# mcahny/vps

Measured on NVIDIA H100. Metric: FuseTrack frame pairs/s on synthetic 1024x2048 pairs, higher is better.
Workload: dtype f32 (wgmma: 3 split-f16 products per MAC, fp32 accumulate promoted to RN register sums)

## Files before the change

vps_b200/csrc/conv_tc32.cu:

```cuda
#include "conv_tc_common.cuh"

namespace {

constexpr int T32_CONV_WARPS = 3;
constexpr int T32_KC = 32;
constexpr int T32_MAX_N = 128;
constexpr int T32_WIDE_MAX_N = 64;
constexpr int t32_threads(int nwg) { return 128 * (nwg + 1); }
constexpr int T32_STAGE_SLOTS = 2;
constexpr int T32_PLANES = 2;

__device__ unsigned int g_tc32_overflow = 0;

struct Tc32Extra {
  int rows;
  int plane_bytes;
  int stage_bytes;
  int b_plane_bytes;
  int dcn;
  int dcn_split_n;
};

constexpr int DCN32_THREADS = 512;
constexpr int DCN32_GATHER_WARPS = 7;
constexpr int DCN32_MAX_N = 128;
constexpr int DCN32_LO_REGS = 80, DCN32_HI_REGS = 176;
static_assert(128 * (2 * DCN32_LO_REGS + 2 * DCN32_HI_REGS) == DCN32_THREADS * (65536 / DCN32_THREADS),
              "the DCN register split must use exactly the launch allocation");
static_assert(DCN32_LO_REGS % 8 == 0 && DCN32_HI_REGS % 8 == 0 && DCN32_LO_REGS >= 24 && DCN32_HI_REGS <= 256,
              "setmaxnreg counts are multiples of 8 in [24, 256]");

struct Ring32 {
  uint32_t s_base, s_bytes;
  uint32_t a_base, a_bytes;
  uint32_t b_base, b_bytes;
  uint32_t e_base, bias_base;
  uint32_t setup_base;
  uint32_t bar_base;
  uint32_t smem;
  __device__ __forceinline__ uint32_t sfull(int s) const { return bar_base + 8u * s; }
  __device__ __forceinline__ uint32_t sempty(int s) const { return bar_base + 8u * (MAX_STAGES + s); }
  __device__ __forceinline__ uint32_t pfull(int s) const { return bar_base + 8u * (2 * MAX_STAGES + s); }
  __device__ __forceinline__ uint32_t pempty(int s) const { return bar_base + 8u * (3 * MAX_STAGES + s); }
  __device__ __forceinline__ uint32_t bfull(int s) const { return bar_base + 8u * (4 * MAX_STAGES + s); }
  __device__ __forceinline__ uint32_t bempty(int s) const { return bar_base + 8u * (5 * MAX_STAGES + s); }
  __device__ __forceinline__ uint32_t unit_ctr() const { return bar_base + 8u * (6 * MAX_STAGES); }
  __device__ __forceinline__ uint32_t rfull(int wg) const { return bar_base + 8u * (6 * MAX_STAGES + 1 + wg); }
};
constexpr int T32_NBAR = 6 * MAX_STAGES;
constexpr int T32_BAR_BYTES = 8 * (T32_NBAR + 2 + 4);
constexpr int t32_box_c(int n) { return n >= 32 ? 32 : 16; }
constexpr int T32_EPI_MAX_N = 64;

__host__ __device__ __forceinline__ Ring32 ring32(uint32_t base, const ConvTcParams& p, const Tc32Extra& e, int nwg, bool epi_tma,
                                                  bool dcn) {
  Ring32 rg;
  rg.s_base = base; rg.s_bytes = dcn ? 0u : (uint32_t)e.stage_bytes;
  rg.a_base = rg.s_base + T32_STAGE_SLOTS * rg.s_bytes; rg.a_bytes = (uint32_t)T32_PLANES * (uint32_t)e.plane_bytes;
  rg.b_base = rg.a_base + (uint32_t)p.a_stages * rg.a_bytes; rg.b_bytes = (uint32_t)T32_PLANES * (uint32_t)e.b_plane_bytes;
  rg.e_base = rg.b_base + (uint32_t)p.b_stages * rg.b_bytes;
  rg.bias_base = rg.e_base + (epi_tma ? 64u * nwg * (uint32_t)p.block_n * 4u : 0u);
  rg.setup_base = rg.bias_base + (epi_tma ? (uint32_t)nwg * (uint32_t)p.block_n * 4u : 0u);
  rg.bar_base = rg.setup_base + (dcn ? (uint32_t)dcn_setup_bytes(e.rows) : 0u);
  rg.smem = rg.bar_base + T32_BAR_BYTES + 1024u - base;
  return rg;
}

struct Tc32Walk {
  int chunks, taps, kw;
  bool halo;
  __host__ __device__ __forceinline__ int steps() const { return chunks * taps; }
  __host__ __device__ __forceinline__ int items() const { return chunks * (halo ? 1 : taps); }
  __device__ __forceinline__ bool opens_item(int tap) const { return !halo || tap == 0; }
};
__host__ __device__ __forceinline__ Tc32Walk tc32_walk(const ConvTcParams& p) { return {p.cin_chunks, p.kh * p.kw, p.kw, p.halo != 0}; }

__device__ __forceinline__ void producer32(const ConvTcParams& p, const Tc32Extra& e, const Ring32& rg, const CUtensorMap* tmA,
                                           const CUtensorMap* tmB) {
  const Tc32Walk walk = tc32_walk(p);
  const uint32_t a_box_bytes = (uint32_t)p.a_box_bytes, b_bytes = (uint32_t)T32_PLANES * (uint32_t)e.b_plane_bytes;
  const int bn = p.block_n;
  RingPos sp, bp;
  for (int tile = blockIdx.x; tile < p.total_tiles; tile += gridDim.x) {
    const TileCoord t = tile_coord(p, tile);
    const int x_base = t.tx * p.tw * p.sw - p.pw_[t.prob];
    const int y_base = t.ty * p.th * p.sh - p.ph_[t.prob];
    const int n0 = t.n_idx * bn;
    for (int cc = 0; cc < walk.chunks; ++cc) {
      for (Tap tap; tap.k < walk.taps; tap.next(walk.kw)) {
        if (!e.dcn && walk.opens_item(tap.k)) {
          sp.wait_empty(rg.sempty(sp.slot));
          if (elect_one()) {
            mbar_expect_tx(rg.sfull(sp.slot), a_box_bytes);
            tma_load_4d(rg.s_base + sp.slot * rg.s_bytes, tmA, rg.sfull(sp.slot), cc * T32_KC,
                        walk.halo ? x_base : x_base + tap.s, walk.halo ? y_base : y_base + tap.r, t.img);
// ... 102 lines not shown
          acc[4] += wq[c] * v1[c].x; acc[5] += wq[c] * v1[c].y; acc[6] += wq[c] * v1[c].z; acc[7] += wq[c] * v1[c].w;
        }
        uint32_t hp[4], lp[4];
        bool over = false;
#pragma unroll
        for (int q = 0; q < 4; ++q) split_pair_f16(acc[2 * q], acc[2 * q + 1], hp[q], lp[q], over);
        if (over) atomicAdd(&g_tc32_overflow, 1u);
        const uint32_t off = (uint32_t)r * 64u + ((((uint32_t)j) ^ ((uint32_t)(r >> 1) & 3u)) << 4);
        const uint32_t pm = dst + off, pl = pm + (uint32_t)e.plane_bytes;
        asm volatile("st.shared.v4.b32 [%0], {%1, %2, %3, %4};" ::"r"(pm), "r"(hp[0]), "r"(hp[1]), "r"(hp[2]), "r"(hp[3]) : "memory");
        asm volatile("st.shared.v4.b32 [%0], {%1, %2, %3, %4};" ::"r"(pl), "r"(lp[0]), "r"(lp[1]), "r"(lp[2]), "r"(lp[3]) : "memory");
      }
      asm volatile("fence.proxy.async.shared::cta;" ::: "memory");
      __syncwarp();
      if (lane == 0) mbar_arrive(rg.pfull(ap.slot));
    }
    step_base += (uint32_t)steps_per_tile;
    asm volatile("bar.sync 1, %0;" ::"n"(NT) : "memory");
  }
}

template <int N>
__device__ __forceinline__ uint32_t epi_box_addr(uint32_t box, int q, int c) {
  constexpr int BC = t32_box_c(N);
  const uint32_t k = (uint32_t)((c % BC) >> 2);
  const uint32_t sw = BC == 32 ? (uint32_t)(q & 7) : (uint32_t)((q >> 1) & 3);
  return box + (uint32_t)(c / BC) * (64u * BC * 4u) + (uint32_t)q * (BC * 4u) + ((k ^ sw) << 4) + (uint32_t)(c & 3) * 4u;
}

struct EpiBox {
  int n0, x0, y0, img;
  bool live;
};
__device__ __forceinline__ EpiBox epi_box(const ConvTcParams& p, int tile, int wg) {
  const TileCoord t = tile_coord(p, tile);
  EpiBox b;
  b.n0 = t.n_idx * p.block_n; b.img = t.img;
  b.x0 = t.tx * p.tw + (64 * wg) % p.tw; b.y0 = t.ty * p.th + (64 * wg) / p.tw;
  b.live = b.x0 < p.ow && b.y0 < p.oh;
  return b;
}

template <int N>
__device__ __forceinline__ void epi_tma32(const ConvTcParams& p, const CUtensorMap* tmY, const float (&d)[N / 2], uint32_t box,
                                          uint32_t bias_s, float bias_v, uint32_t rbar, uint32_t rphase, int wg, int tile) {
  constexpr int BC = t32_box_c(N);
  const int i = threadIdx.x & 127, lane = threadIdx.x & 31, w = i >> 5;
  if (i < N) asm volatile("st.shared.f32 [%0], %1;" ::"r"(bias_s + 4u * i), "f"(bias_v) : "memory");
  if (i == 0) asm volatile("cp.async.bulk.wait_group.read 0;" ::: "memory");
  asm volatile("bar.sync %0, 128;" ::"r"(1 + wg) : "memory");
  if (p.res) mbar_wait(rbar, rphase);
#pragma unroll
  for (int h = 0; h < 2; ++h) {
    const int q = 16 * w + (lane >> 2) + 8 * h;
#pragma unroll
    for (int j = 0; j < N / 8; ++j) {
      const int c = 8 * j + 2 * (lane & 3);
      const uint32_t a = epi_box_addr<N>(box, q, c);
      float b0, b1, r0 = 0.f, r1 = 0.f;
      asm volatile("ld.shared.v2.f32 {%0, %1}, [%2];" : "=f"(b0), "=f"(b1) : "r"(bias_s + 4u * c));
      if (p.res) asm volatile("ld.shared.v2.f32 {%0, %1}, [%2];" : "=f"(r0), "=f"(r1) : "r"(a));
      const float2 v = epi_math(p, d[4 * j + 2 * h], d[4 * j + 2 * h + 1], b0, b1, r0, r1);
      asm volatile("st.shared.v2.f32 [%0], {%1, %2};" ::"r"(a), "f"(v.x), "f"(v.y) : "memory");
    }
  }
  asm volatile("fence.proxy.async.shared::cta;" ::: "memory");
  asm volatile("bar.sync %0, 128;" ::"r"(1 + wg) : "memory");
  const EpiBox eb = epi_box(p, tile, wg);
  if (i == 0 && eb.live) {
#pragma unroll
    for (int b = 0; b < N / BC; ++b) tma_store_4d(tmY, box + (uint32_t)b * (64u * BC * 4u), eb.n0 + b * BC, eb.x0, eb.y0, eb.img);
    asm volatile("cp.async.bulk.commit_group;" ::: "memory");
  }
}

template <int N, bool TMA_EPI>
__device__ __forceinline__ void consumer32(const ConvTcParams& p, const Tc32Extra& e, const Ring32& rg, int wg, int row0,
                                           uint32_t b_off, int c_off, const CUtensorMap* tmY, const CUtensorMap* tmR) {
  constexpr int BC = t32_box_c(N);
  const bool leader = (threadIdx.x & 127) == 0;
  constexpr bool epi_tma = TMA_EPI;
  const uint32_t box = rg.e_base + (uint32_t)wg * (64u * N * 4u), bias_s = rg.bias_base + (uint32_t)wg * (N * 4u);
  const uint32_t rbar = rg.rfull(wg);
  uint32_t rphase = 0;
  const bool halo = p.halo != 0;
  const int ntaps = p.kh * p.kw, kw = p.kw, last_cc = p.cin_chunks - 1;
  const uint32_t a_pitch = halo ? (uint32_t)p.halo_w * 64u : 512u;
  const uint64_t a_hi = desc_hi(64u, a_pitch), b_hi = desc_hi(64u, 512u);
  const uint32_t a_wg = halo ? (uint32_t)(row0 >> 3) * a_pitch : (uint32_t)row0 * 64u;
  const uint32_t plane = (uint32_t)e.plane_bytes, b_plane = (uint32_t)e.b_plane_bytes;
  float acc[N / 2], sum[N / 2];
  RingPos ap, bp;
  for (int tile = blockIdx.x; tile < p.total_tiles; tile += gridDim.x) {
    float bias_v = 0.f;
    if (epi_tma) {
      const int c = tile_coord(p, tile).n_idx * N + (threadIdx.x & 127);
      if (p.bias && (threadIdx.x & 127) < N && c < p.cout) bias_v = __ldg(p.bias + c);
    }
#pragma unroll
    for (int i = 0; i < N / 2; ++i) sum[i] = 0.f;
    for (int cc = 0; cc <= last_cc; ++cc) {
      const bool two = cc != last_cc || p.nk_last > 1;
      uint32_t a_item = 0;
      for (Tap tap; tap.k < ntaps; tap.next(kw)) {
        if (!halo || tap.k == 0) {
          ap.wait_full(rg.pfull(ap.slot));
          a_item = rg.a_base + ap.slot * rg.a_bytes + a_wg;
        }
        bp.wait_full(rg.bfull(bp.slot));
        const uint32_t a_addr = halo ? a_item + (uint32_t)tap.r * a_pitch + (uint32_t)tap.s * 64u : a_item;
        const uint32_t b_addr = rg.b_base + bp.slot * rg.b_bytes + b_off;
        const uint64_t A = desc_at(a_hi, a_addr), A2 = desc_at(a_hi, a_addr + plane);
        const uint64_t B = desc_at(b_hi, b_addr), B2 = desc_at(b_hi, b_addr + b_plane);
        wg::fence();
        wg::Mma<N, true>::run(acc, A2, B, 0u);
        if (two) wg::Mma<N, true>::run(acc, A2 + 2, B + 2, 1u);
        wg::Mma<N, true>::run(acc, A, B2, 1u);
        if (two) wg::Mma<N, true>::run(acc, A + 2, B2 + 2, 1u);
        wg::commit();
        wg::wait<0>();
        wg::fence_regs(acc);
#pragma unroll
        for (int i = 0; i < N / 2; ++i) acc[i] *= T32_LO_INV;
        wg::fence();
        wg::Mma<N, true>::run(acc, A, B, 1u);
        if (two) wg::Mma<N, true>::run(acc, A + 2, B + 2, 1u);
        wg::commit();
        wg::wait<0>();
        wg::fence_regs(acc);
#pragma unroll
        for (int i = 0; i < N / 2; ++i) sum[i] += acc[i];
        const bool item_done = !halo || tap.k == ntaps - 1;
        if (leader) {
          mbar_arrive(rg.bempty(bp.slot));
          if (item_done) mbar_arrive(rg.pempty(ap.slot));
          if (epi_tma && p.res && cc == 0 && tap.k == 0) {
            asm volatile("cp.async.bulk.wait_group.read 0;" ::: "memory");
            const EpiBox eb = epi_box(p, tile, wg);
            if (eb.live) {
              mbar_expect_tx(rbar, 64u * N * 4u);
#pragma unroll
              for (int b = 0; b < N / BC; ++b)
                tma_load_4d(box + (uint32_t)b * (64u * BC * 4u), tmR, rbar, eb.n0 + b * BC, eb.x0, eb.y0, eb.img);
            } else {
              mbar_arrive(rbar);
            }
          }
        }
        ap.next(p.a_stages, item_done);
        bp.next(p.b_stages);
      }
    }
    if (epi_tma) {
      epi_tma32<N>(p, tmY, sum, box, bias_s, bias_v, rbar, rphase, wg, tile);
      if (p.res) rphase ^= 1u;
    } else {
      epi_frag<N, 4>(p, sum, tile, row0, c_off);
    }
  }
  if (epi_tma && leader) asm volatile("cp.async.bulk.wait_group 0;" ::: "memory");
}

template <int NWG, bool TMA_EPI>
__device__ __forceinline__ void consumer32_n(const ConvTcParams& p, const Tc32Extra& e, const Ring32& rg, int wg,
                                             const CUtensorMap* tmY, const CUtensorMap* tmR) {
  switch (p.block_n) {
    case 16: consumer32<16, TMA_EPI>(p, e, rg, wg, 64 * wg, 0u, 0, tmY, tmR); break;
    case 32: consumer32<32, TMA_EPI>(p, e, rg, wg, 64 * wg, 0u, 0, tmY, tmR); break;
    case 64: consumer32<64, TMA_EPI>(p, e, rg, wg, 64 * wg, 0u, 0, tmY, tmR); break;
    default:
      if constexpr (NWG == 2 && !TMA_EPI) consumer32<T32_MAX_N, false>(p, e, rg, wg, 64 * wg, 0u, 0, tmY, tmR);
      else __trap();
      break;
  }
}

__device__ __forceinline__ void init_bars32(const Ring32& rg, uint32_t pfull_count, uint32_t sempty_count, uint32_t consumers) {
  for (int i = threadIdx.x & 31; i < T32_NBAR; i += 32) {
    const int kind = i / MAX_STAGES;
    const uint32_t count = kind == 1 ? sempty_count : (kind == 2 ? pfull_count : ((kind == 3 || kind == 5) ? consumers : 1u));
    mbar_init(rg.bar_base + 8u * i, count);
  }
  if ((threadIdx.x & 31) < 4) mbar_init(rg.rfull(threadIdx.x & 31), 1u);
  asm volatile("fence.mbarrier_init.release.cluster;" ::: "memory");
}

template <int NWG, bool TMA_EPI>
__global__ void __launch_bounds__(t32_threads(NWG), 1)
conv_igemm_tc32_kernel(const __grid_constant__ CUtensorMap tmA, const __grid_constant__ CUtensorMap tmB,
                       const __grid_constant__ CUtensorMap tmY, const __grid_constant__ CUtensorMap tmR, const ConvTcParams p,
                       const Tc32Extra e) {
  extern __shared__ __align__(1024) uint8_t smem_raw[];
  const Ring32 rg = ring32((smem_u32(smem_raw) + 1023u) & ~1023u, p, e, NWG, TMA_EPI, false);
  const int warp = __shfl_sync(0xffffffffu, (int)threadIdx.x >> 5, 0);
  if (warp == 0) init_bars32(rg, 32 * T32_CONV_WARPS, 32 * T32_CONV_WARPS, NWG);
  if (threadIdx.x == 32) {
    asm volatile("prefetch.tensormap [%0];" ::"l"(&tmA) : "memory");
    asm volatile("prefetch.tensormap [%0];" ::"l"(&tmB) : "memory");
    if (TMA_EPI) {
      asm volatile("prefetch.tensormap [%0];" ::"l"(&tmY) : "memory");
      if (p.res) asm volatile("prefetch.tensormap [%0];" ::"l"(&tmR) : "memory");
    }
  }
  __syncthreads();
  asm volatile("griddepcontrol.wait;" ::: "memory");
  asm volatile("griddepcontrol.launch_dependents;" ::: "memory");
  if (warp == 0) producer32(p, e, rg, &tmA, &tmB);
  else if (warp < 4) converter32(p, e, rg, (int)threadIdx.x - 32, 32 * T32_CONV_WARPS);
  else consumer32_n<NWG, TMA_EPI>(p, e, rg, (warp - 4) >> 2, &tmY, &tmR);
}

__global__ void __launch_bounds__(DCN32_THREADS, 1)
dcn_igemm_tc32_kernel(const __grid_constant__ CUtensorMap tmB, const ConvTcParams p, const Tc32Extra e, const DcnParams<float> d) {
  extern __shared__ __align__(1024) uint8_t smem_raw[];
  const Ring32 rg = ring32((smem_u32(smem_raw) + 1023u) & ~1023u, p, e, 2, false, true);
  const int warp = __shfl_sync(0xffffffffu, (int)threadIdx.x >> 5, 0);
  if (warp == 0) init_bars32(rg, (uint32_t)e.rows / 8u, 1, 2);
  if (threadIdx.x == 32) asm volatile("prefetch.tensormap [%0];" ::"l"(&tmB) : "memory");
  __syncthreads();
  asm volatile("griddepcontrol.wait;" ::: "memory");
  asm volatile("griddepcontrol.launch_dependents;" ::: "memory");
  if (warp >= 4 && warp < 12) {
    asm volatile("setmaxnreg.inc.sync.aligned.u32 %0;" ::"n"(DCN32_HI_REGS));
    const int wg = (warp - 4) >> 2;
    const int bn = e.dcn_split_n ? p.block_n / 2 : p.block_n;
    const int row0 = e.dcn_split_n ? 0 : 64 * wg, c_off = e.dcn_split_n ? bn * wg : 0;
    const uint32_t b_off = (uint32_t)c_off * 64u;
    switch (bn) {
      case 16: consumer32<16, false>(p, e, rg, wg, row0, b_off, c_off, nullptr, nullptr); break;
      case 32: consumer32<32, false>(p, e, rg, wg, row0, b_off, c_off, nullptr, nullptr); break;
      case 64: consumer32<64, false>(p, e, rg, wg, row0, b_off, c_off, nullptr, nullptr); break;
      default: consumer32<DCN32_MAX_N, false>(p, e, rg, wg, row0, b_off, c_off, nullptr, nullptr); break;
    }
  } else {
    asm volatile("setmaxnreg.dec.sync.aligned.u32 %0;" ::"n"(DCN32_LO_REGS));
    if (warp == 0) producer32(p, e, rg, &tmB, &tmB);
    else dcn_gather32(p, e, d, rg, rg.setup_base, rg.unit_ctr(), warp < 4 ? (int)threadIdx.x - 32 : (int)threadIdx.x - 384 + 96);
  }
}

__global__ void pack_weights_tc32_kernel(const float* __restrict__ src, const float* __restrict__ scale, unsigned short* __restrict__ bm,
                                         unsigned short* __restrict__ bl, int cout, int cin, int kh, int kw, int cout_pad,
                                         int cin_pad, int transposed) {
  const int64_t total = (int64_t)cout_pad * kh * kw * cin_pad;
  bool over = false;
  for (int64_t i = blockIdx.x * (int64_t)blockDim.x + threadIdx.x; i < total; i += (int64_t)gridDim.x * blockDim.x) {
    const float v = packed_weight(src, scale, i, cout, cin, kh, kw, cin_pad, transposed);
    unsigned short h, l;
    split_f16(v, h, l);
    over = over || f16_over(v);
    bm[i] = h;
    bl[i] = l;
  }
  if (over) atomicAdd(&g_tc32_overflow, 1u);
}

inline int64_t plane_elems(int cout, int cin, int kh, int kw) {
  const int64_t cout_pad = (cout + 15) / 16 * 16, cin_pad = (cin + T32_KC - 1) / T32_KC * T32_KC;
  return cout_pad * kh * kw * cin_pad;
}

bool encode_weights_tc32(CUtensorMap* m, const void* w, int nprob, int cout, int taps, int cin_pad, int block_n, const char* who) {
  const auto encode = vps::tensor_map_encoder();
  if (!encode) return false;
  const int cout_pad = (cout + 15) / 16 * 16;
  const int64_t n_plane = (int64_t)cout_pad * taps * cin_pad;
  cuuint64_t dims[5] = {(cuuint64_t)cin_pad, (cuuint64_t)cout_pad, (cuuint64_t)taps, (cuuint64_t)nprob, T32_PLANES};
  cuuint64_t strides[4] = {(cuuint64_t)taps * cin_pad * 2, (cuuint64_t)cin_pad * 2, (cuuint64_t)n_plane * 2,
                           (cuuint64_t)n_plane * nprob * 2};
  cuuint32_t box[5] = {(cuuint32_t)T32_KC, (cuuint32_t)block_n, 1, 1, T32_PLANES};
  cuuint32_t estr[5] = {1, 1, 1, 1, 1};
  const CUresult r = encode(m, CU_TENSOR_MAP_DATA_TYPE_UINT16, 5, (void*)w, dims, strides, box, estr, CU_TENSOR_MAP_INTERLEAVE_NONE,
                            CU_TENSOR_MAP_SWIZZLE_64B, CU_TENSOR_MAP_L2_PROMOTION_L2_256B, CU_TENSOR_MAP_FLOAT_OOB_FILL_NONE);
  if (r != CUDA_SUCCESS) { vps::set_error("%s: encode B failed (%d)", who, (int)r); return false; }
  return true;
}

constexpr int T32_SMEM_MAX = 227 * 1024 - 64;

struct Tc32Plan {
  ConvTcParams p;
  Tc32Extra e;
  int nwg;
  int epi_tma;
  int smem;
};

bool tc32_epi_expressible(const vps_conv_args* a, int nprob) {
  if (nprob != 1 || a->oy_mul != 1 || a->ox_mul != 1 || a->y.dtype != VPS_F32) return false;
  const int64_t px = (int64_t)a->oy_off * a->y.w + a->ox_off;
  if ((((uintptr_t)a->y.ptr + px * a->y.cs * 4) & 15) || a->y.cs % 4) return false;
  if (a->res.ptr && (a->res.dtype != VPS_F32 || (((uintptr_t)a->res.ptr + px * a->res.cs * 4) & 15) || a->res.cs % 4))
    return false;
  return true;
}

Tc32Plan tc32_tile(const vps_conv_args* a, int nprob, int nwg, int block_n) {
  Tc32Plan g = {};
  ConvTcParams& p = g.p;
  g.nwg = nwg;
  const int px = 64 * nwg;
  p.halo = a->sh == 1 && a->sw == 1 && a->kh * a->kw > 1 && a->kh <= 8 && a->kw <= 8;
  const int tw = p.halo ? 8 : patch_tw(a->oh, a->ow, px, a->sh, a->sw);
  set_tiles(p, a, nprob, tw, px / tw, block_n, T32_KC);
  p.halo_w = tw + a->kw - 1;
  p.a_stages = p.halo ? 2 : 3;
  g.e.rows = p.halo ? (p.th + a->kh - 1) * p.halo_w : px;
  p.a_box_bytes = g.e.rows * 128;
  g.e.stage_bytes = (g.e.rows * 128 + 1023) / 1024 * 1024;
  g.e.plane_bytes = (g.e.rows * 64 + 1023) / 1024 * 1024;
  g.e.b_plane_bytes = block_n * 64;
  return g;
}

int tc32_plan(const vps_conv_args* a, int nprob, Tc32Plan& out) {
  VPS_CHECK_ARG(nprob >= 1 && nprob <= MAX_PROB, "conv2d_tc32: nprob %d", nprob);
  VPS_CHECK_ARG(a->sh >= 1 && a->sh <= 2 && a->sw >= 1 && a->sw <= 2, "conv2d_tc32: stride must be 1 or 2");
  VPS_CHECK_ARG(a->kh >= 1 && a->kw >= 1 && a->cin >= 1 && a->cout >= 1 && a->oh >= 0 && a->ow >= 0 && a->x.n >= 0,
                "conv2d_tc32: bad geometry (k %dx%d, cin %d, cout %d, out %dx%d)", a->kh, a->kw, a->cin, a->cout, a->oh, a->ow);
  const int sms = vps::num_sms();
  if (sms <= 0) { vps::set_error("no device"); return VPS_E_NODEV; }
  const int cout_pad = (a->cout + 15) / 16 * 16;
  double best = -1.0;
  for (int nwg = 2; nwg <= 4; nwg += 2) {
    for (int bn = 16; bn <= (nwg == 2 ? T32_MAX_N : T32_WIDE_MAX_N) && bn <= cout_pad; bn *= 2) {
      if (cout_pad % bn) continue;
      Tc32Plan g = tc32_tile(a, nprob, nwg, bn);
      g.p.b_stages = 2;
      if ((int)ring32(0, g.p, g.e, nwg, false, false).smem > T32_SMEM_MAX) continue;
      const int64_t tiles = g.p.total_tiles;
      const double waves = (double)((tiles + sms - 1) / sms);
      const double conv = 2.0 * (g.p.halo ? (double)g.e.rows / (a->kh * a->kw) : (double)g.e.rows);
      const double step = fmax(fmax(300.0, 1.5 * nwg * bn), fmax((double)(bn * 64 * T32_PLANES) / 56.0, conv));
      const double t = waves * ((double)tc32_walk(g.p).steps() * step + 40.0 * bn + 1500.0);
      if (best < 0 || t < best * 0.999) {
        best = t;
        out = g;
      }
    }
  }
  if (best < 0) {
    vps::set_error("conv2d_tc32: ring does not fit (k %dx%d)", a->kh, a->kw);
    return VPS_E_ARG;
  }
  ConvTcParams& p = out.p;
  p.b_stages = 2;
  const auto epi_fits = [&] { return (int)ring32(0, p, out.e, out.nwg, true, false).smem <= T32_SMEM_MAX; };
  if (!p.halo && p.block_n <= T32_EPI_MAX_N && tc32_epi_expressible(a, nprob)) {
    if (!epi_fits() && p.a_stages == 3) {
      p.a_stages = 2;
      if (!epi_fits()) p.a_stages = 3;
    }
    out.epi_tma = epi_fits();
  }
  p.b_stages = 0;
  const Ring32 rg = ring32(0, p, out.e, out.nwg, out.epi_tma, false);
  const int bst = (T32_SMEM_MAX - (int)rg.smem) / (int)rg.b_bytes;
  p.b_stages = bst > MAX_STAGES ? MAX_STAGES : bst;
  out.smem = (int)ring32(0, p, out.e, out.nwg, out.epi_tma, false).smem;
  return VPS_OK;
}

constexpr int DCN32_SMEM_MAX = 132 * 1024;
constexpr double DCN32_UNIT_CLK = 220.0, DCN32_STEP_CLK = 300.0;

int dcn32_plan(const vps_conv_args* a, Tc32Plan& out) {
  const int sms = vps::num_sms();
  if (sms <= 0) { vps::set_error("no device"); return VPS_E_NODEV; }
  const int cout_pad = (a->cout + 15) / 16 * 16;
  double best = -1.0, best_units = 0.0;
  for (int split_n = 0; split_n <= 1; ++split_n) {
    const int rows = split_n ? 64 : 128;
    const int tw = patch_tw(a->oh, a->ow, rows, 1, 1);
    for (int bn = 16; bn <= DCN32_MAX_N; bn *= 2) {
      const int block_n = split_n ? 2 * bn : bn;
      if (block_n > cout_pad || cout_pad % block_n) continue;
      Tc32Plan g = {};
      set_tiles(g.p, a, 1, tw, rows / tw, block_n, T32_KC);
      g.p.a_stages = 2;
      g.e.rows = rows; g.e.plane_bytes = rows * 64; g.e.b_plane_bytes = block_n * 64; g.e.dcn = 1; g.e.dcn_split_n = split_n;
      const Ring32 rg = ring32(0, g.p, g.e, 2, false, true);
      const int bst = (DCN32_SMEM_MAX - (int)rg.smem) / (int)rg.b_bytes;
      if (bst < 2) continue;
      const int64_t tiles = g.p.total_tiles;
      const double waves = (double)((tiles + sms - 1) / sms);
      const double step = fmax(fmax(rows / 8 * DCN32_UNIT_CLK, fmax(DCN32_STEP_CLK, 6.0 * bn)), rg.b_bytes / 56.0);
      const double t = waves * ((double)tc32_walk(g.p).steps() * step + 40.0 * bn + 1500.0), units = waves * rows;
      if (best < 0 || t < best * 0.999 || (t <= best * 1.001 && units < best_units)) {
        best = t; best_units = units;
        g.p.b_stages = bst > 3 ? 3 : bst;
        g.smem = (int)ring32(0, g.p, g.e, 2, false, true).smem;
        out = g;
      }
    }
  }
  if (best < 0) {
    vps::set_error("deform_conv_tc32: no tiling fits (cout %d)", a->cout);
    return VPS_E_ARG;
  }
  return VPS_OK;
}

}

extern "C" int64_t vps_packed_tc32_bytes(int cout, int cin, int kh, int kw, int nprob) {
  return plane_elems(cout, cin, kh, kw) * 2 * T32_PLANES * nprob;
}

extern "C" unsigned int* vps_tc32_overflow_flag() {
  unsigned int* p = nullptr;
  if (cudaGetSymbolAddress((void**)&p, g_tc32_overflow) != cudaSuccess) return nullptr;
  return p;
}
// ... 24 lines not shown

extern "C" int vps_conv2d_tc32_multi(const vps_conv_args* args, int nprob, void* stream) {
  VPS_CHECK_ARG(nprob >= 1 && nprob <= MAX_PROB, "conv2d_tc32: nprob %d", nprob);
  const vps_conv_args* a = &args[0];
  VPS_CHECK_ARG(a->x.dtype == VPS_F32, "conv2d_tc32: x must be fp32");
  VPS_CHECK_ARG(a->x.cs % 4 == 0 && ((uintptr_t)a->x.ptr & 15) == 0, "conv2d_tc32: x not 16B aligned (cs=%d)", a->x.cs);
  VPS_CHECK_ARG(a->cin == a->x.c, "conv2d_tc32: cin %d != x.c %d", a->cin, a->x.c);
  VPS_CHECK_ARG(((uintptr_t)a->w & 127) == 0, "conv2d_tc32: weights not aligned");
  for (int i = 0; i < nprob; ++i) {
    VPS_CHECK_ARG(args[i].w == a->w && args[i].x.ptr == a->x.ptr && args[i].y.ptr == a->y.ptr && args[i].kh == a->kh &&
                      args[i].kw == a->kw && args[i].oh == a->oh && args[i].ow == a->ow && args[i].cout == a->cout &&
                      args[i].bias == a->bias && args[i].act == a->act && args[i].oy_mul == a->oy_mul && args[i].ox_mul == a->ox_mul,
                  "conv2d_tc32_multi: problems must share geometry and the packed weight buffer");
  }
  Tc32Plan g;
  int st = tc32_plan(a, nprob, g);
  if (st != VPS_OK) return st;
  ConvTcParams& p = g.p;
  const int halo_h = p.th + p.kh - 1;
  VPS_CHECK_ARG(p.b_stages >= 2, "conv2d_tc32: ring does not fit (%d x %d px halo, bn %d)", halo_h, p.halo_w, p.block_n);
  st = set_problems(p, args, nprob, "conv2d_tc32");
  if (st != VPS_OK) return st;
  if (p.total_tiles == 0) return VPS_OK;

  CUtensorMap tmA, tmB;
  if (!vps::encode_nhwc(&tmA, a->x, CU_TENSOR_MAP_DATA_TYPE_FLOAT32, T32_KC, p.halo ? p.halo_w : p.tw * a->sw,
                        p.halo ? halo_h : p.th * a->sh, a->sw, a->sh, CU_TENSOR_MAP_SWIZZLE_128B, CU_TENSOR_MAP_L2_PROMOTION_L2_128B,
                        "conv2d_tc32: encode A"))
    return VPS_E_CUDA;
  if (!encode_weights_tc32(&tmB, a->w, nprob, a->cout, a->kh * a->kw, p.cin_chunks * T32_KC, p.block_n, "conv2d_tc32"))
    return VPS_E_CUDA;
  CUtensorMap tmY = {}, tmR = {};
  if (g.epi_tma) {
    const int bc = t32_box_c(p.block_n), box_w = p.tw < 64 ? p.tw : 64;
    const int64_t px = (int64_t)a->oy_off * a->y.w + a->ox_off;
    for (int m = 0; m < (a->res.ptr ? 2 : 1); ++m) {
      const vps_tensor& t = m ? a->res : a->y;
      vps_tensor v = t;
      v.ptr = (float*)t.ptr + px * t.cs; v.n = a->x.n; v.h = a->oh; v.w = a->ow; v.c = a->cout;
      if (!vps::encode_nhwc(m ? &tmR : &tmY, v, CU_TENSOR_MAP_DATA_TYPE_FLOAT32, bc, box_w, 64 / box_w, 1, 1,
                            bc == 32 ? CU_TENSOR_MAP_SWIZZLE_128B : CU_TENSOR_MAP_SWIZZLE_64B, CU_TENSOR_MAP_L2_PROMOTION_L2_128B,
                            m ? "conv2d_tc32: encode residual" : "conv2d_tc32: encode output", &t))
        return VPS_E_CUDA;
    }
  }
#define VPS_TC32_LAUNCH(NWG, EPI)                                                                                              \
  launch_persistent<conv_igemm_tc32_kernel<NWG, EPI>>(p.total_tiles, t32_threads(NWG), g.smem, stream, "conv2d_tc32", tmA, tmB,  \
                                                      tmY, tmR, p, g.e)
  if (g.nwg == 4) return g.epi_tma ? VPS_TC32_LAUNCH(4, true) : VPS_TC32_LAUNCH(4, false);
  return g.epi_tma ? VPS_TC32_LAUNCH(2, true) : VPS_TC32_LAUNCH(2, false);
#undef VPS_TC32_LAUNCH
}

extern "C" int vps_conv2d_tc32(const vps_conv_args* a, void* stream) { return vps_conv2d_tc32_multi(a, 1, stream); }

extern "C" int vps_conv2d_tc32_plan(const vps_conv_args* a, int nprob, int* plan) {
  Tc32Plan g;
  const int st = tc32_plan(a, nprob, g);
  if (st != VPS_OK) return st;
  plan[0] = g.nwg; plan[1] = g.p.block_n; plan[2] = g.p.tw; plan[3] = g.p.th; plan[4] = g.p.halo; plan[5] = g.epi_tma;
  return VPS_OK;
}


extern "C" int vps_deform_conv_tc32(const vps_tensor* x, const vps_tensor* offset, const void* w, int cout, const vps_tensor* y,
                                    void* stream) {
  VPS_CHECK_ARG(x->dtype == VPS_F32 && offset->dtype == VPS_F32 && offset->c >= 18, "deform_conv_tc32: dtypes");
  VPS_CHECK_ARG(x->c % T32_KC == 0 && x->cs % 8 == 0 && ((uintptr_t)x->ptr & 31) == 0,
                "deform_conv_tc32: x must have cin %% 32 == 0 and 32-byte aligned pixel rows (256-bit sampling loads)");
  VPS_CHECK_ARG(offset->n == x->n && offset->h == x->h && offset->w == x->w && y->n == x->n && y->h == x->h && y->w == x->w &&
                    y->c == cout, "deform_conv_tc32: shapes");
  VPS_CHECK_ARG((int64_t)x->n * x->h * x->w * x->cs < (1ll << 31), "deform_conv_tc32: tensor too large for 32-bit offsets");
  VPS_CHECK_ARG(((uintptr_t)w & 127) == 0, "deform_conv_tc32: weights not aligned");
  VPS_CHECK_ARG(y->dtype == VPS_F32, "deform_conv_tc32: y must be fp32");
  vps_conv_args a = dcn_args(*x, cout);
  a.y = *y;
  Tc32Plan g;
  int st = dcn32_plan(&a, g);
  if (st != VPS_OK) return st;
  st = set_problems(g.p, &a, 1, "deform_conv_tc32");
  if (st != VPS_OK) return st;
  if (g.p.total_tiles == 0) return VPS_OK;
  const DcnParams<float> d = {(const float*)x->ptr, (const float*)offset->ptr, x->cs, offset->cs, x->h, x->w};
  CUtensorMap tmB;
  if (!encode_weights_tc32(&tmB, w, 1, cout, 9, x->c, g.p.block_n, "deform_conv_tc32")) return VPS_E_CUDA;
  static bool carveout_set = false;
  if (!carveout_set) {
    cudaFuncSetAttribute(dcn_igemm_tc32_kernel, cudaFuncAttributePreferredSharedMemoryCarveout, 58);
    (void)cudaGetLastError();
    carveout_set = true;
  }
  return launch_persistent<dcn_igemm_tc32_kernel>(g.p.total_tiles, DCN32_THREADS, g.smem, stream, "deform_conv_tc32", tmB, g.p, g.e,
                                                  d);
}

extern "C" int vps_deform_conv_tc32_plan(const vps_tensor* x, int cout, int* plan) {
  VPS_CHECK_ARG(x->c % T32_KC == 0 && x->c > 0 && cout > 0, "deform_conv_tc32_plan: cin %d, cout %d", x->c, cout);
  const vps_conv_args a = dcn_args(*x, cout);
  Tc32Plan g;
  const int st = dcn32_plan(&a, g);
  if (st != VPS_OK) return st;
  plan[0] = g.e.rows; plan[1] = g.e.dcn_split_n ? g.p.block_n / 2 : g.p.block_n; plan[2] = g.e.dcn_split_n; plan[3] = g.p.n_tiles_n;
  return VPS_OK;
}
```

vps_b200/ops.py:

```python
import ctypes as C
import os

import torch

from . import _lib
from ._lib import (ACT_LRELU, ACT_NONE, ACT_RELU, ACT_SIGMOID, VPS_BF16, VPS_F32, VpsConvArgs, VpsError,
                   VpsTensor, check, lib)

_DT = {torch.float32: VPS_F32, torch.bfloat16: VPS_BF16}

PROFILE = None
_NOTE = {"flops": 0, "tag": ""}
SCOPE = [""]
_real_lib = lib


class _ProfLib(object):
    def __getattr__(self, name):
        f = getattr(_real_lib(), name)
        if PROFILE is None or not name.startswith("vps_") or name in ("vps_last_error", "vps_launch_count", "vps_packed_tc_bytes"):
            return f

        def w(*a):
            s, e = torch.cuda.Event(enable_timing=True), torch.cuda.Event(enable_timing=True)
# ... 190 lines not shown
    else:
        a.w = pw.simt().data_ptr()
        check(lib().vps_conv2d_simt(C.byref(a), stream()), "conv2d_simt")
    return y


def conv2d_tc_multi(x, pws, y, pads, omaps, act=ACT_NONE, slope=0.1, out_scale=1.0, oh=None, ow=None, shared32=None):
    n = len(pws)
    arr = (VpsConvArgs * n)()
    gran = pws[0].gran()
    f32 = x.dtype == torch.float32
    for i in range(n):
        a = _conv_args(x, pws[i], y, 1, 0, act, slope, None, False, out_scale, oh, ow, omaps[i], pads[i])
        a.cin_gran = gran
        a.w = shared32.data_ptr() if f32 else pws[i].tc(gran).data_ptr()
        arr[i] = a
    if PROFILE is not None:
        _NOTE["flops"] = 2 * x.shape[0] * arr[0].oh * arr[0].ow * pws[0].cout * pws[0].cin * arr[0].kh * arr[0].kw * n
        _NOTE["tag"] = "%dx%d x%d phases %d->%d @%dx%d" % (arr[0].kh, arr[0].kw, n, pws[0].cin, pws[0].cout, arr[0].oh, arr[0].ow)
    if f32:
        check(lib().vps_conv2d_tc32_multi(arr, n, stream()), "conv2d_tc32_multi")
    else:
        check(lib().vps_conv2d_tc_multi(arr, n, stream()), "conv2d_tc_multi")
    return y


def conv2d_tc32_plan(x, pws, stride=1, pad=0, oh=None, ow=None, pads=None, y=None, res=None, omaps=None):
    pws = pws if isinstance(pws, (list, tuple)) else [pws]
    n = len(pws)
    arr = (VpsConvArgs * n)()
    for i in range(n):
        arr[i] = _conv_args(x, pws[i], x if y is None else y, stride, pad, ACT_NONE, 0.1, res, False, 1.0, oh, ow,
                            omaps[i] if omaps is not None else (1, 0, 1, 0), pads[i] if pads is not None else None)
    plan = (C.c_int * 6)()
    check(_real_lib().vps_conv2d_tc32_plan(arr, n, plan), "conv2d_tc32_plan")
    return dict(nwg=plan[0], block_n=plan[1], tw=plan[2], th=plan[3], halo=plan[4], epilogue="tma" if plan[5] else "frag")


def conv2d_tc_plan(x, pws, stride=1, pad=0, oh=None, ow=None, pads=None, y=None, res=None, omaps=None):
    pws = pws if isinstance(pws, (list, tuple)) else [pws]
    n = len(pws)
    arr = (VpsConvArgs * n)()
    for i in range(n):
        arr[i] = _conv_args(x, pws[i], x if y is None else y, stride, pad, ACT_NONE, 0.1, res, False, 1.0, oh, ow,
                            omaps[i] if omaps is not None else (1, 0, 1, 0), pads[i] if pads is not None else None)
        arr[i].cin_gran = pws[0].gran()
    plan = (C.c_int * 10)()
    check(_real_lib().vps_conv2d_tc_plan(arr, n, plan), "conv2d_tc_plan")
    keys = ("block_n", "tw", "th", "halo", "rowg", "gsub", "bk", "a_stages", "b_stages", "total_tiles")
    return dict(zip(keys, plan))


def correlation(f1, f2, out, pad, max_disp, stride1, stride2, act=ACT_NONE, slope=0.1, impl=None):
    fn = {None: "vps_correlation", "tc": "vps_correlation_tc", "simt": "vps_correlation_simt", "tc32": "vps_correlation_tc32"}[impl]
    if PROFILE is not None:
        d = 2 * (max_disp // stride2) + 1
        _NOTE["flops"] = 2 * f1.shape[0] * f1.shape[1] * f1.shape[2] * f1.shape[3] * d * d
        _NOTE["tag"] = "corr d%d s%d C%d @%dx%d" % (max_disp, stride2, f1.shape[3], f1.shape[1], f1.shape[2])
    if impl is None and F32_TC[0] and f1.dtype == torch.float32 and f2.dtype == torch.float32 and out.dtype == torch.float32:
        c = f1.shape[3]
        if (c % 64 == 0 and c <= 256 and stride1 == 1 and pad == max_disp and (max_disp, stride2) == (20, 2)
                and vt(f1).cs % 4 == 0 and vt(f2).cs % 4 == 0 and f1.data_ptr() % 16 == 0 and f2.data_ptr() % 16 == 0):
            fn = "vps_correlation_tc32"
    if fn == "vps_correlation_tc32":
        ws = torch.empty(int(lib().vps_correlation_tc32_ws_bytes(C.byref(vt(f1)))), dtype=torch.uint8, device=f1.device)
        off = (-ws.data_ptr()) % 256
        check(lib().vps_correlation_tc32(C.byref(vt(f1)), C.byref(vt(f2)), C.byref(vt(out)), pad, max_disp, stride1, stride2,
                                         act, C.c_float(slope), C.c_void_p(ws.data_ptr() + off), stream()), "correlation_tc32")
        return out
# ... 270 lines not shown
```

vps_b200/synth.py:

```python
import math

import torch
import torch.nn as nn


def _kaiming_uniform(w, gain=1.0):
    fan_in = w[0].numel()
    bound = gain * math.sqrt(3.0 / fan_in)
    w.uniform_(-bound, bound)


@torch.no_grad()
def init_weights(model, kind="C", seed=0):
    g = torch.Generator().manual_seed(seed)

    def U(t, a, b):
        t.copy_(torch.rand(t.shape, generator=g) * (b - a) + a)

    def N(t, mean, std):
        t.copy_(torch.randn(t.shape, generator=g) * std + mean)

    if kind == "A":
        for name, m in model.named_modules():
            if isinstance(m, (nn.Conv2d, nn.ConvTranspose2d, nn.Linear)):
                if name.startswith("flownet2"):
                    fan_in = m.weight[0].numel() if not isinstance(m, nn.ConvTranspose2d) else m.weight.shape[0] * m.weight[0, 0].numel()
                    fan_out = m.weight.shape[0] * m.weight[0, 0].numel() if not isinstance(m, nn.ConvTranspose2d) else m.weight[0].numel()
                    b = math.sqrt(6.0 / (fan_in + fan_out))
                    U(m.weight, -b, b)
                    if m.bias is not None:
                        U(m.bias, 0, 1)
                elif name.startswith("backbone"):
                    fan_out = m.weight.shape[0] * m.weight[0, 0].numel()
                    N(m.weight, 0, math.sqrt(2.0 / fan_out))
                elif name.startswith(("rpn_head", "track_head")):
                    N(m.weight, 0, 0.01); m.bias.zero_()
                elif name == "bbox_head.fc_cls":
                    N(m.weight, 0, 0.01); m.bias.zero_()
                elif name == "bbox_head.fc_reg":
                    N(m.weight, 0, 0.001); m.bias.zero_()
                else:
                    fan_in = m.weight[0].numel()
                    fan_out = m.weight.shape[0] * (m.weight[0, 0].numel() if m.weight.dim() > 2 else 1)
                    b = math.sqrt(6.0 / (fan_in + fan_out))
                    U(m.weight, -b, b)
                    if m.bias is not None:
                        m.bias.zero_()
            elif isinstance(m, nn.BatchNorm2d):
                m.weight.fill_(1); m.bias.zero_(); m.running_mean.zero_(); m.running_var.fill_(1)
                if name.endswith("bn3"):
                    m.weight.zero_()
        return model

    for name, m in model.named_modules():
        if isinstance(m, (nn.Conv2d, nn.Linear)):
            _g = 1.4 if not name.startswith("flownet2") else 1.0
            fan_in = m.weight[0].numel()
            bound = _g * math.sqrt(3.0 / fan_in)
            U(m.weight, -bound, bound)
            if m.bias is not None:
                N(m.bias, 0, 0.05)
        elif isinstance(m, nn.ConvTranspose2d):
            fan_in = m.weight.shape[0] * m.weight[0, 0].numel() / 4.0
            bound = math.sqrt(3.0 / fan_in)
            U(m.weight, -bound, bound)
            if m.bias is not None:
                N(m.bias, 0, 0.05)
        elif isinstance(m, nn.BatchNorm2d):
            U(m.weight, 0.5, 1.5); N(m.bias, 0, 0.1); N(m.running_mean, 0, 0.1); U(m.running_var, 0.5, 1.5)
            if name.endswith("bn3"):
                m.weight.mul_(0.5)
        elif isinstance(m, nn.GroupNorm):
            U(m.weight, 0.5, 1.5); N(m.bias, 0, 0.1)
        elif m.__class__.__name__ in ("DeformConv", "_DeformConv"):
            fan_in = m.weight[0].numel()
            bound = 1.4 * math.sqrt(3.0 / fan_in)
            U(m.weight, -bound, bound)
    for name, m in model.named_modules():
        if name.endswith("conv_offset"):
            N(m.weight, 0, 0.02); N(m.bias, 0, 0.5)
    for name, m in model.named_modules():
        if name.startswith("flownet2") and "predict_flow" in name:
            m.weight.mul_(0.2)
    model.rpn_head.rpn_cls.weight.mul_(2.0)
# ... 53 lines not shown
```

Baseline: 16.61.

## Let tc32 conv split output channels across warpgroups and retune the tile cost model

Generalizes the per-warpgroup work split so the four consumer warpgroups can share one 64-row pixel block and divide the output channels (wg_n of 2 or 4), not only stack pixel rows. This gives tiles with wider block_n (up to 256) that reuse the same A tile across more channels. The planner now searches these layouts with a new clock-based cost model whose constants differ from the old heuristic. The DCN channel-split path is folded into the same mechanism. The cost model may pick layouts that lower occupancy or raise the B-operand shared-memory traffic. A synth.py init tweak for DeformConv weights is also included.

Result: faster. 17.89, median of 6 (+7.7%).

```diff
diff --git a/vps_b200/csrc/conv_tc32.cu b/vps_b200/csrc/conv_tc32.cu
--- a/vps_b200/csrc/conv_tc32.cu
+++ b/vps_b200/csrc/conv_tc32.cu
@@ -18,8 +18,16 @@
   int stage_bytes;
   int b_plane_bytes;
   int dcn;
-  int dcn_split_n;
+  int wg_n;
 };
+
+struct Tc32Share {
+  int row0, c_off, n;
+};
+__host__ __device__ __forceinline__ Tc32Share tc32_share(const ConvTcParams& p, const Tc32Extra& e, int wg) {
+  const int n = p.block_n / e.wg_n, lg = e.wg_n >> 1;
+  return {64 * (wg >> lg), n * (wg & (e.wg_n - 1)), n};
+}
 
 constexpr int DCN32_THREADS = 512;
 constexpr int DCN32_GATHER_WARPS = 7;
@@ -55,12 +63,13 @@
 __host__ __device__ __forceinline__ Ring32 ring32(uint32_t base, const ConvTcParams& p, const Tc32Extra& e, int nwg, bool epi_tma,
                                                   bool dcn) {
   Ring32 rg;
+  const uint32_t n = (uint32_t)(p.block_n / e.wg_n);
   rg.s_base = base; rg.s_bytes = dcn ? 0u : (uint32_t)e.stage_bytes;
   rg.a_base = rg.s_base + T32_STAGE_SLOTS * rg.s_bytes; rg.a_bytes = (uint32_t)T32_PLANES * (uint32_t)e.plane_bytes;
   rg.b_base = rg.a_base + (uint32_t)p.a_stages * rg.a_bytes; rg.b_bytes = (uint32_t)T32_PLANES * (uint32_t)e.b_plane_bytes;
   rg.e_base = rg.b_base + (uint32_t)p.b_stages * rg.b_bytes;
-  rg.bias_base = rg.e_base + (epi_tma ? 64u * nwg * (uint32_t)p.block_n * 4u : 0u);
-  rg.setup_base = rg.bias_base + (epi_tma ? (uint32_t)nwg * (uint32_t)p.block_n * 4u : 0u);
+  rg.bias_base = rg.e_base + (epi_tma ? 64u * nwg * n * 4u : 0u);
+  rg.setup_base = rg.bias_base + (epi_tma ? (uint32_t)nwg * n * 4u : 0u);
   rg.bar_base = rg.setup_base + (dcn ? (uint32_t)dcn_setup_bytes(e.rows) : 0u);
   rg.smem = rg.bar_base + T32_BAR_BYTES + 1024u - base;
   return rg;
@@ -229,17 +238,18 @@
   int n0, x0, y0, img;
   bool live;
 };
-__device__ __forceinline__ EpiBox epi_box(const ConvTcParams& p, int tile, int wg) {
+__device__ __forceinline__ EpiBox epi_box(const ConvTcParams& p, const Tc32Extra& e, int tile, int wg) {
   const TileCoord t = tile_coord(p, tile);
+  const Tc32Share s = tc32_share(p, e, wg);
   EpiBox b;
-  b.n0 = t.n_idx * p.block_n; b.img = t.img;
-  b.x0 = t.tx * p.tw + (64 * wg) % p.tw; b.y0 = t.ty * p.th + (64 * wg) / p.tw;
+  b.n0 = t.n_idx * p.block_n + s.c_off; b.img = t.img;
+  b.x0 = t.tx * p.tw + s.row0 % p.tw; b.y0 = t.ty * p.th + s.row0 / p.tw;
   b.live = b.x0 < p.ow && b.y0 < p.oh;
   return b;
 }
 
 template <int N>
-__device__ __forceinline__ void epi_tma32(const ConvTcParams& p, const CUtensorMap* tmY, const float (&d)[N / 2], uint32_t box,
+__device__ __forceinline__ void epi_tma32(const ConvTcParams& p, const Tc32Extra& e, const CUtensorMap* tmY, const float (&d)[N / 2], uint32_t box,
                                           uint32_t bias_s, float bias_v, uint32_t rbar, uint32_t rphase, int wg, int tile) {
   constexpr int BC = t32_box_c(N);
   const int i = threadIdx.x & 127, lane = threadIdx.x & 31, w = i >> 5;
@@ -263,7 +273,7 @@
   }
   asm volatile("fence.proxy.async.shared::cta;" ::: "memory");
   asm volatile("bar.sync %0, 128;" ::"r"(1 + wg) : "memory");
-  const EpiBox eb = epi_box(p, tile, wg);
+  const EpiBox eb = epi_box(p, e, tile, wg);
   if (i == 0 && eb.live) {
 #pragma unroll
     for (int b = 0; b < N / BC; ++b) tma_store_4d(tmY, box + (uint32_t)b * (64u * BC * 4u), eb.n0 + b * BC, eb.x0, eb.y0, eb.img);
@@ -272,11 +282,13 @@
 }
 
 template <int N, bool TMA_EPI>
-__device__ __forceinline__ void consumer32(const ConvTcParams& p, const Tc32Extra& e, const Ring32& rg, int wg, int row0,
-                                           uint32_t b_off, int c_off, const CUtensorMap* tmY, const CUtensorMap* tmR) {
+__device__ __forceinline__ void consumer32(const ConvTcParams& p, const Tc32Extra& e, const Ring32& rg, int wg, const CUtensorMap* tmY,
+                                           const CUtensorMap* tmR) {
   constexpr int BC = t32_box_c(N);
   const bool leader = (threadIdx.x & 127) == 0;
   constexpr bool epi_tma = TMA_EPI;
+  const Tc32Share s = tc32_share(p, e, wg);
+  const uint32_t b_base = rg.b_base + (uint32_t)s.c_off * 64u;
   const uint32_t box = rg.e_base + (uint32_t)wg * (64u * N * 4u), bias_s = rg.bias_base + (uint32_t)wg * (N * 4u);
   const uint32_t rbar = rg.rfull(wg);
   uint32_t rphase = 0;
@@ -284,14 +296,14 @@
   const int ntaps = p.kh * p.kw, kw = p.kw, last_cc = p.cin_chunks - 1;
   const uint32_t a_pitch = halo ? (uint32_t)p.halo_w * 64u : 512u;
   const uint64_t a_hi = desc_hi(64u, a_pitch), b_hi = desc_hi(64u, 512u);
-  const uint32_t a_wg = halo ? (uint32_t)(row0 >> 3) * a_pitch : (uint32_t)row0 * 64u;
+  const uint32_t a_wg = halo ? (uint32_t)(s.row0 >> 3) * a_pitch : (uint32_t)s.row0 * 64u;
   const uint32_t plane = (uint32_t)e.plane_bytes, b_plane = (uint32_t)e.b_plane_bytes;
   float acc[N / 2], sum[N / 2];
   RingPos ap, bp;
   for (int tile = blockIdx.x; tile < p.total_tiles; tile += gridDim.x) {
     float bias_v = 0.f;
     if (epi_tma) {
-      const int c = tile_coord(p, tile).n_idx * N + (threadIdx.x & 127);
+      const int c = tile_coord(p, tile).n_idx * p.block_n + tc32_share(p, e, wg).c_off + (threadIdx.x & 127);
       if (p.bias && (threadIdx.x & 127) < N && c < p.cout) bias_v = __ldg(p.bias + c);
     }
 #pragma unroll
@@ -306,7 +318,7 @@
         }
         bp.wait_full(rg.bfull(bp.slot));
         const uint32_t a_addr = halo ? a_item + (uint32_t)tap.r * a_pitch + (uint32_t)tap.s * 64u : a_item;
-        const uint32_t b_addr = rg.b_base + bp.slot * rg.b_bytes + b_off;
+        const uint32_t b_addr = b_base + bp.slot * rg.b_bytes;
         const uint64_t A = desc_at(a_hi, a_addr), A2 = desc_at(a_hi, a_addr + plane);
         const uint64_t B = desc_at(b_hi, b_addr), B2 = desc_at(b_hi, b_addr + b_plane);
         wg::fence();
@@ -333,7 +345,7 @@
           if (item_done) mbar_arrive(rg.pempty(ap.slot));
           if (epi_tma && p.res && cc == 0 && tap.k == 0) {
             asm volatile("cp.async.bulk.wait_group.read 0;" ::: "memory");
-            const EpiBox eb = epi_box(p, tile, wg);
+            const EpiBox eb = epi_box(p, e, tile, wg);
             if (eb.live) {
               mbar_expect_tx(rbar, 64u * N * 4u);
 #pragma unroll
@@ -349,10 +361,11 @@
       }
     }
     if (epi_tma) {
-      epi_tma32<N>(p, tmY, sum, box, bias_s, bias_v, rbar, rphase, wg, tile);
+      epi_tma32<N>(p, e, tmY, sum, box, bias_s, bias_v, rbar, rphase, wg, tile);
       if (p.res) rphase ^= 1u;
     } else {
-      epi_frag<N, 4>(p, sum, tile, row0, c_off);
+      const Tc32Share s = tc32_share(p, e, wg);
+      epi_frag<N, 4>(p, sum, tile, s.row0, s.c_off);
     }
   }
   if (epi_tma && leader) asm volatile("cp.async.bulk.wait_group 0;" ::: "memory");
@@ -361,12 +374,12 @@
 template <int NWG, bool TMA_EPI>
 __device__ __forceinline__ void consumer32_n(const ConvTcParams& p, const Tc32Extra& e, const Ring32& rg, int wg,
                                              const CUtensorMap* tmY, const CUtensorMap* tmR) {
-  switch (p.block_n) {
-    case 16: consumer32<16, TMA_EPI>(p, e, rg, wg, 64 * wg, 0u, 0, tmY, tmR); break;
-    case 32: consumer32<32, TMA_EPI>(p, e, rg, wg, 64 * wg, 0u, 0, tmY, tmR); break;
-    case 64: consumer32<64, TMA_EPI>(p, e, rg, wg, 64 * wg, 0u, 0, tmY, tmR); break;
+  switch (p.block_n / e.wg_n) {
+    case 16: consumer32<16, TMA_EPI>(p, e, rg, wg, tmY, tmR); break;
+    case 32: consumer32<32, TMA_EPI>(p, e, rg, wg, tmY, tmR); break;
+    case 64: consumer32<64, TMA_EPI>(p, e, rg, wg, tmY, tmR); break;
     default:
-      if constexpr (NWG == 2 && !TMA_EPI) consumer32<T32_MAX_N, false>(p, e, rg, wg, 64 * wg, 0u, 0, tmY, tmR);
+      if constexpr (NWG == 2 && !TMA_EPI) consumer32<T32_MAX_N, false>(p, e, rg, wg, tmY, tmR);
       else __trap();
       break;
   }
@@ -420,14 +433,11 @@
   if (warp >= 4 && warp < 12) {
     asm volatile("setmaxnreg.inc.sync.aligned.u32 %0;" ::"n"(DCN32_HI_REGS));
     const int wg = (warp - 4) >> 2;
-    const int bn = e.dcn_split_n ? p.block_n / 2 : p.block_n;
-    const int row0 = e.dcn_split_n ? 0 : 64 * wg, c_off = e.dcn_split_n ? bn * wg : 0;
-    const uint32_t b_off = (uint32_t)c_off * 64u;
-    switch (bn) {
-      case 16: consumer32<16, false>(p, e, rg, wg, row0, b_off, c_off, nullptr, nullptr); break;
-      case 32: consumer32<32, false>(p, e, rg, wg, row0, b_off, c_off, nullptr, nullptr); break;
-      case 64: consumer32<64, false>(p, e, rg, wg, row0, b_off, c_off, nullptr, nullptr); break;
-      default: consumer32<DCN32_MAX_N, false>(p, e, rg, wg, row0, b_off, c_off, nullptr, nullptr); break;
+    switch (p.block_n / e.wg_n) {
+      case 16: consumer32<16, false>(p, e, rg, wg, nullptr, nullptr); break;
+      case 32: consumer32<32, false>(p, e, rg, wg, nullptr, nullptr); break;
+      case 64: consumer32<64, false>(p, e, rg, wg, nullptr, nullptr); break;
+      default: consumer32<DCN32_MAX_N, false>(p, e, rg, wg, nullptr, nullptr); break;
     }
   } else {
     asm volatile("setmaxnreg.dec.sync.aligned.u32 %0;" ::"n"(DCN32_LO_REGS));
@@ -492,11 +502,12 @@
   return true;
 }
 
-Tc32Plan tc32_tile(const vps_conv_args* a, int nprob, int nwg, int block_n) {
+Tc32Plan tc32_tile(const vps_conv_args* a, int nprob, int nwg, int wg_n, int n) {
   Tc32Plan g = {};
   ConvTcParams& p = g.p;
   g.nwg = nwg;
-  const int px = 64 * nwg;
+  g.e.wg_n = wg_n;
+  const int px = 64 * (nwg / wg_n), block_n = wg_n * n;
   p.halo = a->sh == 1 && a->sw == 1 && a->kh * a->kw > 1 && a->kh <= 8 && a->kw <= 8;
   const int tw = p.halo ? 8 : patch_tw(a->oh, a->ow, px, a->sh, a->sw);
   set_tiles(p, a, nprob, tw, px / tw, block_n, T32_KC);
@@ -510,6 +521,7 @@
   return g;
 }
 
+constexpr double T32_STEP_CLK = 410.0, T32_STEP_CLK_640 = 70.0, T32_MMA_CLK_N2 = 0.4, T32_CONV_CLK = 6.0, T32_B_BYTES_PER_CLK = 200.0;
 int tc32_plan(const vps_conv_args* a, int nprob, Tc32Plan& out) {
   VPS_CHECK_ARG(nprob >= 1 && nprob <= MAX_PROB, "conv2d_tc32: nprob %d", nprob);
   VPS_CHECK_ARG(a->sh >= 1 && a->sh <= 2 && a->sw >= 1 && a->sw <= 2, "conv2d_tc32: stride must be 1 or 2");
@@ -519,20 +531,24 @@
   if (sms <= 0) { vps::set_error("no device"); return VPS_E_NODEV; }
   const int cout_pad = (a->cout + 15) / 16 * 16;
   double best = -1.0;
-  for (int nwg = 2; nwg <= 4; nwg += 2) {
-    for (int bn = 16; bn <= (nwg == 2 ? T32_MAX_N : T32_WIDE_MAX_N) && bn <= cout_pad; bn *= 2) {
-      if (cout_pad % bn) continue;
-      Tc32Plan g = tc32_tile(a, nprob, nwg, bn);
-      g.p.b_stages = 2;
-      if ((int)ring32(0, g.p, g.e, nwg, false, false).smem > T32_SMEM_MAX) continue;
-      const int64_t tiles = g.p.total_tiles;
-      const double waves = (double)((tiles + sms - 1) / sms);
-      const double conv = 2.0 * (g.p.halo ? (double)g.e.rows / (a->kh * a->kw) : (double)g.e.rows);
-      const double step = fmax(fmax(300.0, 1.5 * nwg * bn), fmax((double)(bn * 64 * T32_PLANES) / 56.0, conv));
-      const double t = waves * ((double)tc32_walk(g.p).steps() * step + 40.0 * bn + 1500.0);
-      if (best < 0 || t < best * 0.999) {
-        best = t;
-        out = g;
+  for (int wg_n = 1; wg_n <= 4; wg_n *= 2) {
+    for (int nwg = 2; nwg <= 4; nwg += 2) {
+      if (wg_n > 1 && nwg == 2) continue;
+      for (int n = 16; n <= (nwg == 2 ? T32_MAX_N : T32_WIDE_MAX_N) && wg_n * n <= cout_pad; n *= 2) {
+        if (cout_pad % (wg_n * n) || (wg_n > 1 && n != T32_WIDE_MAX_N)) continue;
+        Tc32Plan g = tc32_tile(a, nprob, nwg, wg_n, n);
+        g.p.b_stages = 2;
+        if ((int)ring32(0, g.p, g.e, nwg, false, false).smem > T32_SMEM_MAX) continue;
+        const int64_t tiles = g.p.total_tiles;
+        const double waves = (double)((tiles + sms - 1) / sms);
+        const double rows = g.p.halo ? (double)g.e.rows / (a->kh * a->kw) : (double)g.e.rows;
+        const double step = T32_STEP_CLK + (nwg == 4 ? T32_STEP_CLK_640 : T32_MMA_CLK_N2 * n) + 3.0 * nwg * n + T32_CONV_CLK * rows +
+                            (double)(g.p.block_n * 64 * T32_PLANES) / T32_B_BYTES_PER_CLK;
+        const double t = waves * ((double)tc32_walk(g.p).steps() * step + 40.0 * n + 1500.0);
+        if (best < 0 || t < best * 0.999) {
+          best = t;
+          out = g;
+        }
       }
     }
   }
@@ -543,7 +559,7 @@
   ConvTcParams& p = out.p;
   p.b_stages = 2;
   const auto epi_fits = [&] { return (int)ring32(0, p, out.e, out.nwg, true, false).smem <= T32_SMEM_MAX; };
-  if (!p.halo && p.block_n <= T32_EPI_MAX_N && tc32_epi_expressible(a, nprob)) {
+  if (!p.halo && p.block_n / out.e.wg_n <= T32_EPI_MAX_N && tc32_epi_expressible(a, nprob)) {
     if (!epi_fits() && p.a_stages == 3) {
       p.a_stages = 2;
       if (!epi_fits()) p.a_stages = 3;
@@ -575,7 +591,7 @@
       Tc32Plan g = {};
       set_tiles(g.p, a, 1, tw, rows / tw, block_n, T32_KC);
       g.p.a_stages = 2;
-      g.e.rows = rows; g.e.plane_bytes = rows * 64; g.e.b_plane_bytes = block_n * 64; g.e.dcn = 1; g.e.dcn_split_n = split_n;
+      g.e.rows = rows; g.e.plane_bytes = rows * 64; g.e.b_plane_bytes = block_n * 64; g.e.dcn = 1; g.e.wg_n = split_n ? 2 : 1;
       const Ring32 rg = ring32(0, g.p, g.e, 2, false, true);
       const int bst = (DCN32_SMEM_MAX - (int)rg.smem) / (int)rg.b_bytes;
       if (bst < 2) continue;
@@ -666,7 +682,7 @@
     return VPS_E_CUDA;
   CUtensorMap tmY = {}, tmR = {};
   if (g.epi_tma) {
-    const int bc = t32_box_c(p.block_n), box_w = p.tw < 64 ? p.tw : 64;
+    const int bc = t32_box_c(p.block_n / g.e.wg_n), box_w = p.tw < 64 ? p.tw : 64;
     const int64_t px = (int64_t)a->oy_off * a->y.w + a->ox_off;
     for (int m = 0; m < (a->res.ptr ? 2 : 1); ++m) {
       const vps_tensor& t = m ? a->res : a->y;
@@ -693,6 +709,7 @@
   const int st = tc32_plan(a, nprob, g);
   if (st != VPS_OK) return st;
   plan[0] = g.nwg; plan[1] = g.p.block_n; plan[2] = g.p.tw; plan[3] = g.p.th; plan[4] = g.p.halo; plan[5] = g.epi_tma;
+  plan[6] = g.e.wg_n;
   return VPS_OK;
 }
 
@@ -734,6 +751,6 @@
   Tc32Plan g;
   const int st = dcn32_plan(&a, g);
   if (st != VPS_OK) return st;
-  plan[0] = g.e.rows; plan[1] = g.e.dcn_split_n ? g.p.block_n / 2 : g.p.block_n; plan[2] = g.e.dcn_split_n; plan[3] = g.p.n_tiles_n;
+  plan[0] = g.e.rows; plan[1] = g.p.block_n / g.e.wg_n; plan[2] = g.e.wg_n == 2; plan[3] = g.p.n_tiles_n;
   return VPS_OK;
 }
diff --git a/vps_b200/ops.py b/vps_b200/ops.py
--- a/vps_b200/ops.py
+++ b/vps_b200/ops.py
@@ -246,9 +246,10 @@
     for i in range(n):
         arr[i] = _conv_args(x, pws[i], x if y is None else y, stride, pad, ACT_NONE, 0.1, res, False, 1.0, oh, ow,
                             omaps[i] if omaps is not None else (1, 0, 1, 0), pads[i] if pads is not None else None)
-    plan = (C.c_int * 6)()
+    plan = (C.c_int * 7)()
     check(_real_lib().vps_conv2d_tc32_plan(arr, n, plan), "conv2d_tc32_plan")
-    return dict(nwg=plan[0], block_n=plan[1], tw=plan[2], th=plan[3], halo=plan[4], epilogue="tma" if plan[5] else "frag")
+    return dict(nwg=plan[0], block_n=plan[1], tw=plan[2], th=plan[3], halo=plan[4], epilogue="tma" if plan[5] else "frag",
+                wg_n=plan[6], layout=(plan[0] // plan[6], plan[6]))
 
 
 def conv2d_tc_plan(x, pws, stride=1, pad=0, oh=None, ow=None, pads=None, y=None, res=None, omaps=None):
diff --git a/vps_b200/synth.py b/vps_b200/synth.py
--- a/vps_b200/synth.py
+++ b/vps_b200/synth.py
@@ -50,6 +50,9 @@
                 m.weight.fill_(1); m.bias.zero_(); m.running_mean.zero_(); m.running_var.fill_(1)
                 if name.endswith("bn3"):
                     m.weight.zero_()
+            elif m.__class__.__name__ in ("DeformConv", "_DeformConv"):
+                stdv = 1.0 / math.sqrt(m.weight[0].numel())
+                U(m.weight, -stdv, stdv)
         return model
 
     for name, m in model.named_modules():
```
